# Kevindqz/hybrid-vehicle-platoon

Hardware: NVIDIA B200
Metric: hybrid-MPC solves/sec at n=10,N=6 (per-vehicle local MIQPs, proven optimal) (higher is better)
Workload: dtype f64

## Files before the change

hybrid_vehicle_platoon_b200/csrc/flat_core.cuh:

```cuda
#pragma once
#include <math.h>
#include <stdint.h>

#include "miqp_core.cuh"

#if defined(__CUDACC__)
#define HVP_ROLL _Pragma("unroll 1")
#define HVP_FLAT_UNROLL _Pragma("unroll")
#else
#define HVP_ROLL
#define HVP_FLAT_UNROLL
#endif
#if defined(__CUDA_ARCH__)
#define HVP_LDG(p) __ldg(p)
#else
#define HVP_LDG(p) (*(p))
#endif

namespace hvp {

#if defined(__CUDA_ARCH__)
extern __shared__ double hvp_flat_slab[];
#endif

HVP_HD double hvp_rcp(double v) {
#if defined(__CUDA_ARCH__)
    double r;
    asm("rcp.approx.ftz.f64 %0, %1;" : "=d"(r) : "d"(v));
    r = r * (2.0 - v * r);
    r = r * (2.0 - v * r);
    return r;
#else
    return 1.0 / v;
#endif
}

#ifdef HVP_DEBUG_STATS
static long g_it[16], g_nodes[16], g_q[16], g_st[4], g_warm[8];
#endif
template <int N>
struct FlatLayout {
    static constexpr int TRI = N * (N + 1) / 2;
    static constexpr int O_HINV = 0;
    static constexpr int O_GINV = N * N;
    static constexpr int O_X = O_GINV + TRI;
    static constexpr int O_LAM = O_X + N;
    static constexpr int O_YP = O_LAM + N;
    static constexpr int O_D = O_YP + N;
    static constexpr int O_WV = O_D;
    static constexpr int O_R = O_D + N;
    static constexpr int SIZE = O_R + N;
};

template <int N>
struct FlatCold {
    double gt[N], xstar[N], rlo[N + 1], rhi[N + 1], amax[N], amin[N];
    long long t_start;
    double pf[N + 1], pnz[N + 1], ptp[N + 1], ptm[N + 1];
};

template <int N, int ST, bool ALG2 = false, bool HINTS = false>
struct FlatSolver {
    using LY = FlatLayout<N>;
    enum : int { S_NEXT = 0, S_BUILD, S_SELECT, S_STEP, S_DONE };
    static constexpr bool kHull = false;

    double* W;
    const LocalParams* P;
    const double* xf_;
    const double* xb_;
    double* best_;
    FlatCold<N>* C;
    double p0, v0, pc, inv_m, a_lo, a_hi, c_lo, c_hi, hw1, hw2, hd, ct;
    bool has_sf, has_sb;
    double sfv[N], sbv[N];
    int state, lev, L, nodes, iters, it;
    double inc;
    uint64_t modes_pk, best_modes, cand_pk, built_pk;
    int built_L;
    bool trouble, limit, timeout;
    bool dive;
    bool hinted;
    int hint_c0;
    bool fresh;
#ifdef HVP_DEBUG_STATS
    bool was_warm = false;
#endif
    bool slab_ok;
    int q;
    uint64_t act_lo, act_hi;
    uint32_t satf, satb;
    int pid, pkind, pj;
    double psgn, pcoef, nHn, lam_p, cp;
    double dual;
    bool p_soft;

    int lane_;
    HVP_HD double& w(int off, int i) const {
#if defined(__CUDA_ARCH__)
        return hvp_flat_slab[(off + i) * ST + lane_];
#else
        return W[(size_t)(off + i) * ST];
#endif
    }
    HVP_HD static int tri(int a, int b) { return a * (a + 1) / 2 + b; }
    HVP_HD double ra(int rg) const { return rg < 4 ? a_lo : a_hi; }
    HVP_HD double rc(int rg) const { return rg < 4 ? c_lo : c_hi; }
    HVP_HD double rb(int rg) const { return P->bgear[rg] * inv_m; }
    HVP_HD static int mode_of(uint64_t pk, int k) { return (int)((pk >> (3 * k)) & 7u); }
    HVP_HD int mode(int k) const { return mode_of(modes_pk, k); }
    HVP_HD void set_mode(int k, int rg) { modes_pk = (modes_pk & ~(7ull << (3 * k))) | ((uint64_t)rg << (3 * k)); }
    HVP_HD int cand(int lv) const { return (int)((cand_pk >> (7 * lv)) & 0x7fu); }
    HVP_HD void set_cand(int lv, int v) { cand_pk = (cand_pk & ~(0x7full << (7 * lv))) | ((uint64_t)v << (7 * lv)); }
    HVP_HD int act_raw(int a) const { return (int)(((a < 8 ? act_lo >> (8 * a) : act_hi >> (8 * (a - 8)))) & 0xffu); }
    HVP_HD int act(int a) const { return act_raw(a) & 0x7f; }
    HVP_HD double slot_sgn(int a) const { return (act_raw(a) & 0x80) ? -1.0 : 1.0; }
    HVP_HD double slot_coef(int a) const {
        const int id = act(a), t = id / 12;
        return (t == T_UHI || t == T_ULO) ? ra(mode(id - 12 * t)) : 1.0;
    }
    HVP_HD void set_act(int a, int id) {
        if (a < 8) act_lo = (act_lo & ~(0xffull << (8 * a))) | ((uint64_t)id << (8 * a));
        else act_hi = (act_hi & ~(0xffull << (8 * (a - 8)))) | ((uint64_t)id << (8 * (a - 8)));
    }
    HVP_HD double Hoff(int j) const { return hw1 * (double)(N - 1 - j) + hw2; }
    HVP_HD double Hdiag(int j) const { return hw1 * (double)(N - 1 - j) + hd; }
    HVP_HD double sf(int j) const { return HVP_LDG(xf_ + j + 1) - P->d_safe - pc; }
    HVP_HD double sb(int j) const { return HVP_LDG(xb_ + j + 1) + P->d_safe - pc; }

    HVP_HD void setup(double* W_, const LocalParams* P_, int flags, double mass, const double* x0,
                      const double* xf, const double* xb, const double* xl, double* best_out, FlatCold<N>* cold) {
        W = W_; P = P_; xf_ = xf; xb_ = xb; best_ = best_out; C = cold;
        p0 = x0[0]; v0 = x0[1]; pc = p0 + v0;
        inv_m = hvp_rcp(mass);
        a_lo = 1.0 - P->c1 * inv_m; a_hi = 1.0 - P->c2 * inv_m;
        c_lo = -P->mug; c_hi = -P->mug - P->dfr * inv_m;
        const bool is_front = flags & 1, is_leader = flags & 2, is_trailer = flags & 4;
        const bool tf = !is_front && !is_leader, tb = !is_trailer && !is_leader, tl = is_leader;
        const double wp = P->qxp, wvv = P->qxv, t0 = P->t0, d0 = P->d0;
        const int np1 = N + 1;
        const double nterm = (tf ? 1.0 : 0.0) + (tb ? 1.0 : 0.0) + (tl ? 1.0 : 0.0);
        hw1 = 2.0 * wp * nterm;
        hw2 = 2.0 * wp * (tf ? t0 : 0.0);
        hd = 2.0 * wp * (tf ? t0 * t0 : 0.0) + 2.0 * wvv * nterm;
        HVP_ROLL
        for (int j = 0; j < N; ++j) C->gt[j] = 0.0;
        ct = 0.0;
        HVP_ROLL
        for (int kind = 0; kind < 3; ++kind) {
            const double* ref = kind == 0 ? xf : (kind == 1 ? xb : xl);
            const bool on = kind == 0 ? tf : (kind == 1 ? tb : tl);
            if (!on) continue;
            const double tau = kind == 0 ? t0 : 0.0;
            double suffix = 0.0;
            HVP_ROLL
            for (int k = N; k >= 0; --k) {
                const double pk = ref[k], vk = ref[np1 + k];
                const double Pk = (kind == 0) ? (pk - d0) : (kind == 1) ? (pk + t0 * vk + d0) : pk;
                if (k >= 1) {
                    const double rho = pc - Pk;
                    C->gt[k - 1] += 2.0 * wp * (suffix + tau * rho) - 2.0 * wvv * vk;
                    ct += wp * rho * rho + wvv * vk * vk;
                    suffix += rho;
                } else {
                    const double e0 = p0 + tau * v0 - Pk, e1 = v0 - vk;
                    ct += wp * e0 * e0 + wvv * e1 * e1;
                }
            }
        }
        has_sf = !is_front; has_sb = !is_trailer;
        const double ww = P->w, ds = P->d_safe;
        if (has_sf) {
            const double s0 = p0 - (xf[0] - ds), s1 = pc - (xf[1] - ds);
            ct += ww * (s0 > 0 ? s0 : 0.0) + ww * (s1 > 0 ? s1 : 0.0);
        }
        if (has_sb) {
            const double s0 = (xb[0] + ds) - p0, s1 = (xb[1] + ds) - pc;
            ct += ww * (s0 > 0 ? s0 : 0.0) + ww * (s1 > 0 ? s1 : 0.0);
        }
        HVP_FLAT_UNROLL
        for (int j = 1; j < N; ++j) {
            sfv[j] = has_sf ? sf(j) : 0.0;
            sbv[j] = has_sb ? sb(j) : 0.0;
        }
        sfv[0] = sbv[0] = 0.0;
        if (nterm > 0.5) {
            const double* h0 = P->h0inv[tf ? (tb ? 2 : 1) : 0];
            HVP_ROLL
            for (int e = 0; e < N * N; ++e) w(LY::O_HINV, e) = h0[e];
        } else {
            HVP_ROLL
            for (int i = 0; i < N; ++i) {
                HVP_ROLL
                for (int j = 0; j < N; ++j) w(LY::O_HINV, i * N + j) = (i == j) ? Hdiag(i) : Hoff(i > j ? i : j);
            }
            HVP_ROLL
            for (int k = 0; k < N; ++k) {
                const double pinv = hvp_rcp(w(LY::O_HINV, k * N + k));
                HVP_ROLL
                for (int j = 0; j < N; ++j) w(LY::O_HINV, k * N + j) *= pinv;
                w(LY::O_HINV, k * N + k) = pinv;
                HVP_ROLL
                for (int i = 0; i < N; ++i) {
                    if (i == k) continue;
                    const double f = w(LY::O_HINV, i * N + k);
                    HVP_ROLL
                    for (int j = 0; j < N; ++j)
                        w(LY::O_HINV, i * N + j) = (j == k) ? -f * pinv : w(LY::O_HINV, i * N + j) - f * w(LY::O_HINV, k * N + j);
                }
            }
        }
        built_L = 0; built_pk = 0;
        iters = 0; nodes = 0; it = 0; modes_pk = 0; best_modes = 0; cand_pk = 0;
        inc = HUGE_VAL; trouble = limit = timeout = false; lev = 0; dive = P->dive != 0; fresh = false; slab_ok = false;
        hinted = false;
        if (P->time_limit_ns > 0) C->t_start = hvp_now_ns();
        if (ALG2) C->pf[0] = -HUGE_VAL;
        int c0 = 0;
        HVP_ROLL
        for (int rg = 0; rg < NREG; ++rg)
            if (v0 >= P->edge[rg] && v0 <= P->edge[rg + 1]) c0 |= (1 << rg);
        set_cand(0, c0);
        C->xstar[0] = v0; C->rlo[0] = v0; C->rhi[0] = v0;
        state = S_NEXT;
    }

    HVP_HD void apply_hint(const int32_t* h) {
        const double eps = 1e-9;
        const int c0 = cand(0);
        bool ok = true;
        HVP_ROLL
        for (int lv = 0; lv < N && ok; ++lv) {
            const int rg = h[lv];
            int cn = c0;
            if (lv > 0) {
                cn = 0;
                HVP_ROLL
                for (int c = 0; c < NREG; ++c)
                    if (P->edge[c] <= C->rhi[lv] && P->edge[c + 1] >= C->rlo[lv]) cn |= (1 << c);
            }
            if (rg < 0 || rg >= NREG || !((cn >> rg) & 1)) { ok = false; break; }
            set_mode(lv, rg);
            set_cand(lv, cn & ~(1 << rg));
            const double jlo = fmax(C->rlo[lv], P->edge[rg]), jhi = fmin(C->rhi[lv], P->edge[rg + 1]);
            double nlo = fmax(ra(rg) * jlo + rc(rg) + rb(rg) * P->umin, jlo + P->a_dec + lv * P->tight);
            double nhi = fmin(ra(rg) * jhi + rc(rg) + rb(rg) * P->umax, jhi + P->a_acc - lv * P->tight);
            nlo = fmax(nlo, P->vmin); nhi = fmin(nhi, P->vmax);
            if (jlo > jhi + eps || nlo > nhi + eps) { ok = false; break; }
            if (lv + 1 < N) { C->rlo[lv + 1] = nlo - eps; C->rhi[lv + 1] = nhi + eps; C->xstar[lv + 1] = v0; }
        }
        if (!ok || pc > P->pmax + eps || pc < P->pmin - eps) { unhint(c0); return; }
        hint_c0 = c0;
        lev = N - 1;
        L = N;
        hinted = true;
        state = S_BUILD;
    }
    HVP_HD void unhint(int c0) {
        modes_pk = 0; cand_pk = 0;
        set_cand(0, c0);
        lev = 0;
        state = S_NEXT;
    }

    HVP_HD bool open_level(int& l, int& cb, int& total) const {
        l = -1; cb = 0; total = 0;
        HVP_ROLL
        for (int lv = 0; lv <= lev; ++lv) {
            const int c = cand(lv);
            if (c && l < 0) { l = lv; cb = c; }
            total += __builtin_popcount((unsigned)c);
        }
        return l >= 0;
    }
    HVP_HD void adopt_prefix(uint64_t donor_modes, int l, int c, double donor_inc) {
        const double eps = 1e-9;
        HVP_ROLL
        for (int lv = 0; lv < l; ++lv) {
            const int rg = mode_of(donor_modes, lv);
            set_mode(lv, rg);
            set_cand(lv, 0);
            const double jlo = fmax(C->rlo[lv], P->edge[rg]), jhi = fmin(C->rhi[lv], P->edge[rg + 1]);
            double nlo = fmax(ra(rg) * jlo + rc(rg) + rb(rg) * P->umin, jlo + P->a_dec + lv * P->tight);
            double nhi = fmin(ra(rg) * jhi + rc(rg) + rb(rg) * P->umax, jhi + P->a_acc - lv * P->tight);
            nlo = fmax(nlo, P->vmin); nhi = fmin(nhi, P->vmax);
            C->rlo[lv + 1] = nlo - eps; C->rhi[lv + 1] = nhi + eps;
            C->xstar[lv + 1] = v0;
            if (ALG2) C->pf[lv + 1] = -HUGE_VAL;
        }
        fresh = false; slab_ok = false;
        set_cand(l, 1 << c);
        lev = l;
        inc = donor_inc;
        dive = false;
        state = S_NEXT;
    }

    HVP_HD void parent_info() {
        const double ww = P->w, INF = HUGE_VAL;
        const int pj0 = lev - 1;
        HVP_ROLL
        for (int i = 0; i < N; ++i) w(LY::O_YP, i) = w(LY::O_HINV, pj0 * N + i);
        const double nHn0 = w(LY::O_HINV, pj0 * N + pj0);
        HVP_ROLL
        for (int a = 0; a < q; ++a) w(LY::O_D, a) = slot_dot(a, LY::O_YP);
        double nz = nHn0, tp = INF, tm = INF;
        HVP_ROLL
        for (int a = 0; a < q; ++a) {
            double s = 0.0;
            int gi = tri(a, 0);
            HVP_ROLL
            for (int b = 0; b <= a; ++b) s += w(LY::O_GINV, gi + b) * w(LY::O_D, b);
            gi += 2 * a + 1;
            HVP_ROLL
            for (int b = a + 1; b < q; ++b) { s += w(LY::O_GINV, gi) * w(LY::O_D, b); gi += b + 1; }
            nz -= s * w(LY::O_D, a);
            const double la = w(LY::O_LAM, a);
            const bool soft = act(a) >= T_SF * 12;
            if (s > 1e-14) {
                const double is = hvp_rcp(s);
                tp = fmin(tp, la * is);
                if (soft) tm = fmin(tm, (ww - la) * is);
            } else if (s < -1e-14) {
                const double is = hvp_rcp(-s);
                tm = fmin(tm, la * is);
                if (soft) tp = fmin(tp, (ww - la) * is);
            }
        }
        if (q == N || !(nz > 1e-11 * nHn0)) nz = 0.0;
        C->pnz[lev] = nz; C->ptp[lev] = fmax(tp, 0.0); C->ptm[lev] = fmax(tm, 0.0);
    }

    HVP_HD void do_next() {
        const double eps = 1e-9;
        if (ALG2 && fresh) { parent_info(); fresh = false; }
        for (;;) {
            int cset = cand(lev);
            if (cset == 0) {
                if (lev == 0) { state = S_DONE; return; }
                --lev;
                continue;
            }
            int rg = -1; double bd = HUGE_VAL;
            const double xs = C->xstar[lev];
            HVP_ROLL
            for (int c = 0; c < NREG; ++c) {
                if (!((cset >> c) & 1)) continue;
                const double lo = P->edge[c], hi = P->edge[c + 1];
                const double dist = xs < lo ? lo - xs : (xs > hi ? xs - hi : 0.0);
                if (dist < bd) { bd = dist; rg = c; }
            }
            set_cand(lev, cset & ~(1 << rg));
            const double pf = ALG2 ? C->pf[lev] : -HUGE_VAL;
            if (ALG2 && bd > 0.0 && inc < HUGE_VAL && pf > -HUGE_VAL && P->sibling_bound) {
                const double nz = C->pnz[lev];
                const double tmax = (xs > P->edge[rg + 1]) ? C->ptp[lev] : C->ptm[lev];
                const double t = (nz > 0.0) ? fmin(bd * hvp_rcp(nz), tmax) : tmax;
                const double bound = (t < HUGE_VAL) ? pf + t * bd - 0.5 * t * t * nz : HUGE_VAL;
                if (bound > inc) continue;
            }
            set_mode(lev, rg);
            const double jlo = fmax(C->rlo[lev], P->edge[rg]), jhi = fmin(C->rhi[lev], P->edge[rg + 1]);
            if (jlo > jhi + eps) continue;
            double nlo = fmax(ra(rg) * jlo + rc(rg) + rb(rg) * P->umin, jlo + P->a_dec + lev * P->tight);
            double nhi = fmin(ra(rg) * jhi + rc(rg) + rb(rg) * P->umax, jhi + P->a_acc - lev * P->tight);
            nlo = fmax(nlo, P->vmin); nhi = fmin(nhi, P->vmax);
            if (nlo > nhi + eps) continue;
            if (pc > P->pmax + eps || pc < P->pmin - eps) continue;
            C->rlo[lev + 1] = nlo - eps; C->rhi[lev + 1] = nhi + eps;
            L = lev + 1;
            if (dive && nodes >= 1 && L < N) {
                ++lev;
                C->xstar[lev] = w(LY::O_X, lev - 1);
                if (ALG2) C->pf[lev] = -HUGE_VAL;
                int cn = 0;
                HVP_ROLL
                for (int c = 0; c < NREG; ++c)
                    if (P->edge[c] <= C->rhi[lev] && P->edge[c + 1] >= C->rlo[lev]) cn |= (1 << c);
                set_cand(lev, cn);
                continue;
            }
            if (kHull) hull();
            state = S_BUILD;
            return;
        }
    }

    HVP_HD void hull() {
        const double eps = 1e-9;
        double lo = C->rlo[L], hi = C->rhi[L];
        HVP_ROLL
        for (int s = L; s < N; ++s) {
            double nlo = HUGE_VAL, nhi = -HUGE_VAL, dmax = -HUGE_VAL, dmin = HUGE_VAL;
            HVP_ROLL
            for (int r = 0; r < NREG; ++r) {
                const double jlo = fmax(lo, P->edge[r]), jhi = fmin(hi, P->edge[r + 1]);
                if (jlo > jhi + eps) continue;
                const double a = ra(r), b = rb(r), c = rc(r);
                nlo = fmin(nlo, a * jlo + c + b * P->umin);
                nhi = fmax(nhi, a * jhi + c + b * P->umax);
                dmax = fmax(dmax, (a - 1.0) * jlo + c + b * P->umax);
                dmin = fmin(dmin, (a - 1.0) * jhi + c + b * P->umin);
            }
            const double acc = P->a_acc - s * P->tight, dec = P->a_dec + s * P->tight;
            C->amax[s] = fmin(dmax + eps, acc); C->amin[s] = fmax(dmin - eps, dec);
            nlo = fmax(fmax(nlo, lo + dec), P->vmin); nhi = fmin(fmin(nhi, hi + acc), P->vmax);
            lo = nlo - eps; hi = nhi + eps;
            C->rlo[s + 1] = lo; C->rhi[s + 1] = hi;
        }
    }

    HVP_HD void node_done(int st, double obj) {
        iters += it;
        ++nodes;
#ifdef HVP_DEBUG_STATS
        g_it[L] += it; g_nodes[L] += 1; g_q[L] += q; g_st[st] += 1;
        if (was_warm) { g_warm[3] += it; } else { g_warm[4] += it; g_warm[5] += 1; } was_warm = false;
#endif
        state = S_NEXT;
        if (HINTS && hinted) {
            hinted = false;
            if (st != 0) { --nodes; unhint(hint_c0); return; }
            HVP_ROLL
            for (int lv = 1; lv < N; ++lv) C->xstar[lv] = w(LY::O_X, lv - 1);
        }
        if (st != 0 || L == N) dive = false;
        if (st == 2) { trouble = true; return; }
        if (st == 1) return;
        if (inc < HUGE_VAL && !(obj < hvp_cut(inc, P->mip_gap))) return;
        if (L == N) {
            inc = obj; best_modes = modes_pk;
            HVP_ROLL
            for (int j = 0; j < N; ++j) best_[j] = w(LY::O_X, j);
            return;
        }
        if (P->max_nodes > 0 && nodes >= P->max_nodes) { limit = true; state = S_DONE; return; }
        if (P->time_limit_ns > 0 && hvp_now_ns() - C->t_start > P->time_limit_ns) { timeout = true; state = S_DONE; return; }
        ++lev;
        C->xstar[lev] = w(LY::O_X, lev - 1);
        if (ALG2) { C->pf[lev] = fmin(obj, dual); fresh = true; slab_ok = true; }
        int cn = 0;
        HVP_ROLL
        for (int c = 0; c < NREG; ++c)
            if (P->edge[c] <= C->rhi[lev] && P->edge[c + 1] >= C->rlo[lev]) cn |= (1 << c);
        set_cand(lev, cn);
    }

    HVP_HD double rank1(int k, int rg, double s) {
        const double ib = hvp_rcp(rb(rg)), ea = (k >= 1) ? -ra(rg) * ib : 0.0;
        double ev = 0.0;
        HVP_ROLL
        for (int i = 0; i < N; ++i) {
            double v = ib * w(LY::O_HINV, i * N + k);
            if (k >= 1) v += ea * w(LY::O_HINV, i * N + k - 1);
            w(LY::O_WV, i) = v;
        }
        ev = ib * w(LY::O_WV, k) + ((k >= 1) ? ea * w(LY::O_WV, k - 1) : 0.0);
        const double den = hvp_rcp(1.0 / (2.0 * P->qu) * s + ev);
        double vr[N];
        HVP_FLAT_UNROLL
        for (int j = 0; j < N; ++j) vr[j] = w(LY::O_WV, j);
        HVP_ROLL
        for (int i = 0; i < N; ++i) {
            const double vi = w(LY::O_WV, i) * den;
            HVP_FLAT_UNROLL
            for (int j = 0; j < N; ++j) w(LY::O_HINV, i * N + j) -= vi * vr[j];
        }
        return den;
    }

    HVP_HD void do_build() {
        const double qu = P->qu, ww = P->w;
        int c = 0;
        while (c < built_L && c < L && mode_of(built_pk, c) == mode(c)) ++c;
        const bool warm = ALG2 && slab_ok && P->warm && L == built_L + 1 && c == built_L && (satf | satb) == 0u && q > 0;
        slab_ok = false;
        if (warm) {
            const double den = rank1(L - 1, mode(L - 1), 1.0);
            HVP_ROLL
            for (int a = 0; a < q; ++a) w(LY::O_R, a) = slot_dot(a, LY::O_WV);
            double zr = 0.0;
            HVP_ROLL
            for (int a = 0; a < q; ++a) {
                double s = 0.0;
                int gi = tri(a, 0);
                HVP_ROLL
                for (int b = 0; b <= a; ++b) s += w(LY::O_GINV, gi + b) * w(LY::O_R, b);
                gi += 2 * a + 1;
                HVP_ROLL
                for (int b = a + 1; b < q; ++b) { s += w(LY::O_GINV, gi) * w(LY::O_R, b); gi += b + 1; }
                w(LY::O_YP, a) = s;
                zr += s * w(LY::O_R, a);
            }
            const double alpha = den * hvp_rcp(1.0 - den * zr);
            HVP_ROLL
            for (int a = 0; a < q; ++a) {
                const double ra_ = alpha * w(LY::O_YP, a);
                HVP_ROLL
                for (int b = 0; b <= a; ++b) w(LY::O_GINV, tri(a, b)) += ra_ * w(LY::O_YP, b);
            }
        } else {
            HVP_ROLL
            for (int k = built_L - 1; k >= c; --k) rank1(k, mode_of(built_pk, k), -1.0);
            HVP_ROLL
            for (int k = c; k < L; ++k) rank1(k, mode(k), 1.0);
        }
        built_L = L; built_pk = modes_pk;
        HVP_ROLL
        for (int i = 0; i < N; ++i) w(LY::O_D, i) = C->gt[i];
        dual = ct;
        HVP_ROLL
        for (int k = 0; k < L; ++k) {
            const int rg = mode(k);
            const double ib = hvp_rcp(rb(rg)), ea = -ra(rg) * ib;
            const double kc = (k == 0) ? -(ra(rg) * v0 + rc(rg)) * ib : -rc(rg) * ib;
            w(LY::O_D, k) += 2.0 * qu * kc * ib;
            if (k >= 1) w(LY::O_D, k - 1) += 2.0 * qu * kc * ea;
            dual += qu * kc * kc;
        }
        double gr[N];
        HVP_FLAT_UNROLL
        for (int j = 0; j < N; ++j) gr[j] = w(LY::O_D, j);
        HVP_ROLL
        for (int i = 0; i < N; ++i) {
            double s = 0.0;
            HVP_FLAT_UNROLL
            for (int j = 0; j < N; ++j) s -= w(LY::O_HINV, i * N + j) * gr[j];
            if (ALG2) w(LY::O_R, i) = s - w(LY::O_X, i);
            w(LY::O_X, i) = s;
            dual += 0.5 * w(LY::O_D, i) * s;
        }
        it = 0; satf = 0; satb = 0;
        state = S_SELECT;
#ifdef HVP_DEBUG_STATS
        g_warm[0] += 1; if (warm) g_warm[1] += 1;
#endif
        if (warm) {
            HVP_ROLL
            for (int a = 0; a < q; ++a) {
                const int id = act(a), t = id / 12, j = id - 12 * t;
                double cv;
                if (t <= T_LB) {
                    double lo, hi;
                    bounds(j, lo, hi);
                    cv = (t == T_UB) ? w(LY::O_X, j) - hi : lo - w(LY::O_X, j);
                } else {
                    cv = slot_dot(a, LY::O_R);
                }
                w(LY::O_YP, a) = cv;
            }
            bool ok = true;
            double cl = 0.0;
            HVP_ROLL
            for (int a = 0; a < q; ++a) {
                double s = 0.0;
                int gi = tri(a, 0);
                HVP_ROLL
                for (int b = 0; b <= a; ++b) s += w(LY::O_GINV, gi + b) * w(LY::O_YP, b);
// ... 248 lines not shown
            const double is = hvp_rcp(nz);
            HVP_ROLL
            for (int a = 0; a < q; ++a) {
                const double ra_ = w(LY::O_R, a) * is;
                HVP_ROLL
                for (int b = 0; b <= a; ++b) w(LY::O_GINV, tri(a, b)) += ra_ * w(LY::O_R, b);
                w(LY::O_GINV, tri(q, a)) = -ra_;
            }
            w(LY::O_GINV, tri(q, q)) = is;
            set_act(q, pid | (psgn < 0.0 ? 0x80 : 0));
            w(LY::O_LAM, q) = lam_p;
            ++q;
            state = S_SELECT;
            return;
        }
        if (t == t3p) {
            if (pid / 12 == T_SF) satf ^= (1u << pj); else satb ^= (1u << pj);
            state = S_SELECT;
            return;
        }
        int drop;
        if (t == t1) drop = k1;
        else {
            drop = k3;
            const int id = act(drop), j = id % 12;
            if (id / 12 == T_SF) satf ^= (1u << j); else satb ^= (1u << j);
        }
        {
            const double ikk = hvp_rcp(w(LY::O_GINV, tri(drop, drop)));
            HVP_ROLL
            for (int a = 0; a < q; ++a) w(LY::O_D, a) = w(LY::O_GINV, a >= drop ? tri(a, drop) : tri(drop, a));
            HVP_ROLL
            for (int a = 0; a < q; ++a) {
                if (a == drop) continue;
                const int an = a > drop ? a - 1 : a;
                const double da = w(LY::O_D, a) * ikk;
                HVP_ROLL
                for (int b = 0; b <= a; ++b) {
                    if (b == drop) continue;
                    const int bn = b > drop ? b - 1 : b;
                    w(LY::O_GINV, tri(an, bn)) = w(LY::O_GINV, tri(a, b)) - da * w(LY::O_D, b);
                }
            }
        }
        HVP_ROLL
        for (int a = drop; a + 1 < q; ++a) {
            set_act(a, act_raw(a + 1));
            w(LY::O_LAM, a) = w(LY::O_LAM, a + 1);
        }
        --q;
    }

    HVP_HD void trip() {
        if (state == S_NEXT) do_next();
        if (state == S_BUILD) do_build();
        if (state == S_SELECT) do_select();
        if (state == S_STEP) do_step();
    }
    HVP_HD bool wants_node() const { return state == S_NEXT || state == S_BUILD; }
    HVP_HD void trip_node() {
        if (state == S_NEXT) do_next();
        if (state == S_BUILD) do_build();
    }
    HVP_HD void trip_step() {
        if (state == S_SELECT) do_select();
        if (state == S_STEP) do_step();
    }

    HVP_HD LocalResult finish(double* u_out, double* x_out, int32_t* mode_out) const {
        LocalResult R;
        R.nodes = nodes; R.qp_iters = iters;
        const int np1 = N + 1;
        if (inc < HUGE_VAL) {
            R.obj = inc;
            R.status = timeout ? HVP_ST_TIME_LIMIT : limit ? HVP_ST_NODE_LIMIT : (trouble ? HVP_ST_NUMERIC : HVP_ST_OPTIMAL);
            double p = p0, v = v0;
            x_out[0] = p; x_out[np1] = v;
            HVP_ROLL
            for (int k = 0; k < N; ++k) {
                const int rg = mode_of(best_modes, k);
                const double vn = x_out[np1 + k + 1];
                u_out[k] = (vn - ra(rg) * v - rc(rg)) / rb(rg);
                mode_out[k] = rg;
                p = p + v; v = vn;
                x_out[k + 1] = p;
            }
        } else {
            R.obj = HUGE_VAL;
            R.status = timeout ? HVP_ST_TIME_LIMIT : limit ? HVP_ST_NODE_LIMIT : (trouble ? HVP_ST_NUMERIC : HVP_ST_INFEASIBLE);
            HVP_ROLL
            for (int k = 0; k < N; ++k) { u_out[k] = 0.0; mode_out[k] = -1; }
            HVP_ROLL
            for (int k = 0; k <= N; ++k) { x_out[k] = 0.0; x_out[np1 + k] = 0.0; }
        }
        return R;
    }
};

}
```

hybrid_vehicle_platoon_b200/csrc/local_miqp.cu:

```cuda
#include <cuda_runtime.h>
#include <stdint.h>
#include <stdlib.h>
#include <string.h>

#include "coop_core.cuh"
#include "flat_core.cuh"
#include "hvp_internal.h"
#include "miqp_core.cuh"

namespace hvp {

template <int G>
__global__ void __launch_bounds__(COOP_BLOCK)
coop_miqp_kernel(const __grid_constant__ LocalParams P, int64_t batch, const int32_t* __restrict__ flags,
                 const double* __restrict__ mass, const double* __restrict__ x0,
                 const double* __restrict__ xf, const double* __restrict__ xb,
                 const double* __restrict__ xl, double* __restrict__ u, double* __restrict__ x,
                 int32_t* __restrict__ modes, double* __restrict__ obj, int32_t* __restrict__ status,
                 int32_t* __restrict__ nodes, int32_t* __restrict__ qp_iters, int spread) {
    const int64_t t = (int64_t)blockIdx.x * blockDim.x + threadIdx.x;
    if (spread && (threadIdx.x & 31) >= G) return;
    const int64_t i = spread ? (t >> 5) : t / G;
    if (i >= batch) return;
    const int N = P.N;
    const size_t S = 2 * (size_t)(N + 1);
    CoopSolver<DevBK<G>> sol;
    sol.setup(&P, flags[i], mass[i], x0 + 2 * i, xf ? xf + S * i : nullptr, xb ? xb + S * i : nullptr,
              xl ? xl + S * i : nullptr);
    const LocalResult R = sol.solve(u + (size_t)N * i, x + S * i, modes + (size_t)N * i);
    if (sol.bk.ln == 0) {
        obj[i] = R.obj;
        status[i] = R.status;
        nodes[i] = R.nodes;
        if (qp_iters) qp_iters[i] = R.qp_iters;
    }
}

constexpr int COOP_SPLIT_MAX = 64;
constexpr int COOP_SPLIT_ROW = 48;

template <int G>
__global__ void __launch_bounds__(32)
coop_split_kernel(const __grid_constant__ LocalParams P, int64_t batch, int M, const int32_t* __restrict__ flags,
                  const double* __restrict__ mass, const double* __restrict__ x0,
                  const double* __restrict__ xf, const double* __restrict__ xb,
                  const double* __restrict__ xl, double* __restrict__ u, double* __restrict__ x,
                  int32_t* __restrict__ modes, double* __restrict__ obj, int32_t* __restrict__ status,
                  int32_t* __restrict__ nodes, int32_t* __restrict__ qp_iters, unsigned* __restrict__ done,
                  unsigned long long* __restrict__ keys, double* __restrict__ rows) {
    if (threadIdx.x >= G) return;
    const int64_t i = blockIdx.x / M;
    const int w = blockIdx.x % M;
    const int N = P.N, np1 = N + 1;
    const size_t S = 2 * (size_t)np1;
    CoopSolver<DevBK<G>> sol;
    sol.setup(&P, flags[i], mass[i], x0 + 2 * i, xf ? xf + S * i : nullptr, xb ? xb + S * i : nullptr,
              xl ? xl + S * i : nullptr);
    sol.sub_M = M; sol.sub_w = w; sol.shared = keys + i;
    double* row = rows + ((size_t)i * M + w) * COOP_SPLIT_ROW;
    int32_t* rmodes = reinterpret_cast<int32_t*>(row + N + S);
    const LocalResult R = sol.solve(row, row + N, rmodes);
    const int ln = sol.bk.ln;
    unsigned old = 0;
    if (ln == 0) {
        double* tail = row + 2 * N + S;
        tail[0] = R.obj; tail[1] = (double)R.status; tail[2] = (double)R.nodes; tail[3] = (double)R.qp_iters;
    }
    __syncwarp((1u << G) - 1u);
    __threadfence();
    if (ln == 0) old = atomicAdd(done + i, 1u);
    old = __shfl_sync((1u << G) - 1u, old, 0);
    if (old != (unsigned)(M - 2)) return;
    __threadfence();
    double bv = HUGE_VAL;
    int bw = 0, nsum = 0, isum = 0;
    bool numeric = false, limited = false, timed = false;
    for (int c = 0; c < M; ++c) {
        const double* t = rows + ((size_t)i * M + c) * COOP_SPLIT_ROW + 2 * N + S;
        const double o = *reinterpret_cast<const volatile double*>(t);
        const int st = (int)*reinterpret_cast<const volatile double*>(t + 1);
        nsum += (int)*reinterpret_cast<const volatile double*>(t + 2);
        isum += (int)*reinterpret_cast<const volatile double*>(t + 3);
        if (o < bv) { bv = o; bw = c; }
        numeric = numeric || st == HVP_ST_NUMERIC; limited = limited || st == HVP_ST_NODE_LIMIT;
        timed = timed || st == HVP_ST_TIME_LIMIT;
    }
    const double* src = rows + ((size_t)i * M + bw) * COOP_SPLIT_ROW;
    const int32_t* smodes = reinterpret_cast<const int32_t*>(src + N + S);
    for (int e = ln; e < N; e += G) { u[(size_t)N * i + e] = src[e]; modes[(size_t)N * i + e] = smodes[e]; }
    for (int e = ln; e < (int)S; e += G) x[S * i + e] = src[N + e];
    if (ln == 0) {
        obj[i] = bv;
        status[i] = timed ? HVP_ST_TIME_LIMIT : limited ? HVP_ST_NODE_LIMIT
                          : (numeric ? HVP_ST_NUMERIC : (bv < HUGE_VAL ? HVP_ST_OPTIMAL : HVP_ST_INFEASIBLE));
        nodes[i] = nsum;
        if (qp_iters) qp_iters[i] = isum;
    }
}

template <int N, bool STEAL, bool HINTS>
__global__ void __launch_bounds__(32, (N <= 6 ? 10 : (N == 7 ? 7 : (N == 8 ? 6 : 5))))
flat_miqp_kernel(const __grid_constant__ LocalParams P, int64_t batch, const int32_t* __restrict__ flags,
                 const double* __restrict__ mass, const double* __restrict__ x0,
                 const double* __restrict__ xf, const double* __restrict__ xb,
                 const double* __restrict__ xl, double* __restrict__ u, double* __restrict__ x,
                 int32_t* __restrict__ modes, double* __restrict__ obj, int32_t* __restrict__ status,
                 int32_t* __restrict__ nodes, int32_t* __restrict__ qp_iters, unsigned long long* __restrict__ counter,
                 double* __restrict__ scratch) {
    extern __shared__ double smem[];
    using Solver = FlatSolver<N, 32, false, HINTS>;
    const int lane = threadIdx.x;
    const size_t S = 2 * (size_t)(N + 1);
    Solver sol;
    FlatCold<N> cold;
    sol.lane_ = lane;
    sol.P = &P;
    bool have = false;
    int64_t i = 0;
    const bool steal = STEAL && scratch != nullptr && P.max_nodes == 0;
    bool thief = false, drained = false;
    int owner = lane, pending = 0;
    double* const my_scratch = scratch ? scratch + ((size_t)blockIdx.x * 32 + lane) * N : nullptr;
    const int node_batch = P.node_batch;
    for (;;) {
        __syncwarp();
        const bool slow = !have || sol.state == Solver::S_DONE || sol.wants_node();
        const unsigned ms = __ballot_sync(0xffffffffu, slow);
        if (ms == 0xffffffffu || __popc(ms) >= node_batch) {
            if (STEAL && __builtin_expect(drained, 0)) {
                unsigned rep = __ballot_sync(0xffffffffu, have && thief && sol.state == Solver::S_DONE && pending == 0);
                while (rep) {
                    const int r = __ffs(rep) - 1;
                    rep &= rep - 1;
                    const int o = __shfl_sync(0xffffffffu, owner, r);
                    const double v = __shfl_sync(0xffffffffu, sol.inc, r);
                    const unsigned long long bm = __shfl_sync(0xffffffffu, (unsigned long long)sol.best_modes, r);
                    const int nn = __shfl_sync(0xffffffffu, sol.nodes, r), ii = __shfl_sync(0xffffffffu, sol.iters, r);
                    const int tr = __shfl_sync(0xffffffffu, (int)sol.trouble, r);
                    __syncwarp();
                    if (lane == o) {
                        --pending;
                        sol.nodes += nn; sol.iters += ii;
                        if (tr) sol.trouble = true;
                        if (v < sol.inc) {
                            sol.inc = v; sol.best_modes = bm;
                            const double* src = scratch + ((size_t)blockIdx.x * 32 + r) * N;
                            for (int j = 0; j < N; ++j) sol.best_[j] = src[j];
                        }
                    }
                    if (lane == r) { have = false; thief = false; owner = lane; }
                }
                __syncwarp();
            }
            if (have && !thief && sol.state == Solver::S_DONE && pending == 0) {
                const LocalResult R = sol.finish(u + (size_t)N * i, x + S * i, modes + (size_t)N * i);
                obj[i] = R.obj;
                status[i] = R.status;
                nodes[i] = R.nodes;
                if (qp_iters) qp_iters[i] = R.qp_iters;
                have = false;
            }
            bool start = false, adopting = false;
            int a_l = 0, a_c = 0, a_owner = lane;
            unsigned long long a_modes = 0;
            double a_inc = 0.0;
            const unsigned need = __ballot_sync(0xffffffffu, !have);
            if (need && !drained) {
                unsigned long long base = 0;
                if (lane == 0) base = atomicAdd(counter, (unsigned long long)__popc(need));
                base = __shfl_sync(0xffffffffu, base, 0);
                if (!have) {
                    const int64_t cand_i = (int64_t)base + __popc(need & ((1u << lane) - 1u));
                    if (cand_i < batch) { i = cand_i; start = true; }
                }
                if ((int64_t)base + __popc(need) > batch) drained = true;
            }
            if (STEAL && __builtin_expect(steal && drained, 0)) {
                const double oi = __shfl_sync(0xffffffffu, sol.inc, thief ? owner : lane);
                if (have && thief && oi < sol.inc) sol.inc = oi;
                unsigned idle = __ballot_sync(0xffffffffu, !have && !start);
                int l = -1, cb = 0, total = 0;
                const bool can = have && sol.state == Solver::S_NEXT && sol.open_level(l, cb, total) && total >= 2;
                unsigned don = __ballot_sync(0xffffffffu, can);
                for (int round = 0; round < 4 && don && idle; ++round) {
                    const int d = __ffs(don) - 1;
                    don &= don - 1;
                    const int dl = __shfl_sync(0xffffffffu, l, d), dcb = __shfl_sync(0xffffffffu, cb, d);
                    const int dtot = __shfl_sync(0xffffffffu, total, d);
                    const long long di = __shfl_sync(0xffffffffu, (long long)i, d);
                    const unsigned long long dm = __shfl_sync(0xffffffffu, (unsigned long long)sol.modes_pk, d);
                    const double dinc = __shfl_sync(0xffffffffu, sol.inc, d);
                    int m = __popc((unsigned)dcb) - (dtot == __popc((unsigned)dcb) ? 1 : 0);
                    if (m > __popc(idle)) m = __popc(idle);
                    if (m <= 0) continue;
                    const bool me_idle = (idle >> lane) & 1u;
                    const int rk = __popc(idle & ((1u << lane) - 1u));
                    if (me_idle && rk < m) {
                        int bits = dcb;
                        for (int t = 0; t < rk; ++t) bits &= bits - 1;
                        a_c = __ffs(bits) - 1; a_l = dl; a_modes = dm; a_inc = dinc; a_owner = d;
                        i = di; start = true; adopting = true;
                    }
                    if (lane == d) {
                        int bits = dcb, rm = 0;
                        for (int t = 0; t < m; ++t) { rm |= bits & -bits; bits &= bits - 1; }
                        sol.set_cand(dl, dcb & ~rm);
                        pending += m;
                    }
                    idle = __ballot_sync(0xffffffffu, !have && !start);
                }
            }
            if (start) {
                sol.setup(smem + lane, &P, flags[i], mass[i], x0 + 2 * i, xf ? xf + S * i : nullptr,
                          xb ? xb + S * i : nullptr, xl ? xl + S * i : nullptr,
                          adopting ? my_scratch : x + S * i + (N + 2), &cold);
                if (STEAL && adopting) sol.adopt_prefix(a_modes, a_l, a_c, a_inc);
                else if (HINTS && P.hint) sol.apply_hint(P.hint + (size_t)N * i);
                have = true; thief = adopting; owner = a_owner;
            }
            if (!__any_sync(0xffffffffu, have)) break;
            if (have) sol.trip_node();
        }
        if (have) sol.trip_step();
    }
}

static int env_int(const char* name, int dflt) {
    const char* e = getenv(name);
    return e ? atoi(e) : dflt;
}

template <int N>
static cudaError_t launch_flat(const LocalParams& P, unsigned long long* counter, double* steal_scratch, int64_t batch, const int32_t* flags, const double* mass,
                               const double* x0, const double* xf, const double* xb, const double* xl, double* u,
                               double* x, int32_t* modes, double* obj, int32_t* status, int32_t* nodes,
                               int32_t* qp_iters, cudaStream_t stream) {
    const size_t smem = (size_t)FlatLayout<N>::SIZE * 32 * sizeof(double);
    int dev = 0;
    cudaGetDevice(&dev);
    static int grid_cache[HVP_MAX_DEVICES] = {0};
    int uncached = 0;
    int& grid_full = (dev >= 0 && dev < HVP_MAX_DEVICES) ? grid_cache[dev] : uncached;
    if (!grid_full) {
        cudaError_t e = cudaSuccess;
        const void* fns[3] = {(const void*)flat_miqp_kernel<N, true, false>, (const void*)flat_miqp_kernel<N, false, false>,
                              (const void*)flat_miqp_kernel<N, true, true>};
        for (int v = 0; v < 3; ++v) {
            const void* fn = fns[v];
            e = cudaFuncSetAttribute(fn, cudaFuncAttributeMaxDynamicSharedMemorySize, (int)smem);
            if (e != cudaSuccess) return e;
            e = cudaFuncSetAttribute(fn, cudaFuncAttributePreferredSharedMemoryCarveout, cudaSharedmemCarveoutMaxShared);
            if (e != cudaSuccess) return e;
        }
        int sms = 0, per_sm = 0;
        cudaDeviceGetAttribute(&sms, cudaDevAttrMultiProcessorCount, dev);
        e = cudaOccupancyMaxActiveBlocksPerMultiprocessor(&per_sm, flat_miqp_kernel<N, true, false>, 32, smem);
        if (e != cudaSuccess) return e;
        grid_full = sms * (per_sm > 0 ? per_sm : 1);
    }
    int64_t g = (batch + 31) / 32;
    static const int gdiv = env_int("HVP_FLAT_GRID_DIV", 1);
    if (g > grid_full / gdiv) g = grid_full / gdiv;
    LocalParams Q = P;
    static const int nb = env_int("HVP_NODE_BATCH", 0), dv = env_int("HVP_FLAT_DIVE", -1);
    if (nb > 0) Q.node_batch = nb;
    if (dv >= 0) Q.dive = dv;
    static const int steal_on = env_int("HVP_FLAT_STEAL", 1);
    if ((size_t)g * 32 * N > HVP_STEAL_SLOT_DOUBLES) steal_scratch = nullptr;
    cudaError_t e = cudaMemsetAsync(counter, 0, sizeof(unsigned long long), stream);
    if (e != cudaSuccess) return e;
    if (Q.hint)
        flat_miqp_kernel<N, true, true><<<(unsigned)g, 32, smem, stream>>>(Q, batch, flags, mass, x0, xf, xb, xl, u, x, modes, obj,
                                                                          status, nodes, qp_iters, counter,
                                                                          steal_on ? steal_scratch : nullptr);
    else if (steal_on && steal_scratch)
        flat_miqp_kernel<N, true, false><<<(unsigned)g, 32, smem, stream>>>(Q, batch, flags, mass, x0, xf, xb, xl, u, x, modes, obj,
                                                                           status, nodes, qp_iters, counter, steal_scratch);
    else
        flat_miqp_kernel<N, false, false><<<(unsigned)g, 32, smem, stream>>>(Q, batch, flags, mass, x0, xf, xb, xl, u, x, modes, obj,
                                                                            status, nodes, qp_iters, counter, nullptr);
    return cudaGetLastError();
}

static int kernel_choice() {
    static int v = -1;
    if (v < 0) {
        const char* e = getenv("HVP_LOCAL_KERNEL");
        v = 0;
        if (e && strcmp(e, "coop") == 0) v = 2;
        if (e && strcmp(e, "flat") == 0) v = 3;
    }
    return v;
}

cudaError_t launch_local_miqp(const LocalParams& P, unsigned long long* counter, double* steal_scratch, int64_t batch, const int32_t* flags, const double* mass,
                              const double* x0, const double* xf, const double* xb, const double* xl,
                              double* u, double* x, int32_t* modes, double* obj, int32_t* status,
                              int32_t* nodes, int32_t* qp_iters, cudaStream_t stream) {
    if (batch <= 0) return cudaSuccess;
    const int choice = kernel_choice();
    const bool flat_ok = P.N >= 4 && P.N <= 9;
    if (flat_ok && (choice == 3 || (choice == 0 && batch >= FLAT_MIN_BATCH))) {
#define HVP_FLAT(NN) case NN: return launch_flat<NN>(P, counter, steal_scratch, batch, flags, mass, x0, xf, xb, xl, u, x, modes, obj, status, nodes, qp_iters, stream);
        switch (P.N) { HVP_FLAT(4) HVP_FLAT(5) HVP_FLAT(6) HVP_FLAT(7) HVP_FLAT(8) HVP_FLAT(9) default: break; }
#undef HVP_FLAT
    }
    {
        static const int splitM = env_int("HVP_COOP_SPLIT_M", 8);
        if (P.N <= 8 && batch <= COOP_SPLIT_MAX && splitM > 1 && splitM <= 32 && steal_scratch && P.max_nodes == 0 &&
            2 * P.N + 2 * (P.N + 1) + 4 <= COOP_SPLIT_ROW) {
            const size_t head = (size_t)COOP_SPLIT_MAX * (sizeof(unsigned) + sizeof(unsigned long long));
            unsigned* done = reinterpret_cast<unsigned*>(steal_scratch);
            unsigned long long* keys = reinterpret_cast<unsigned long long*>(reinterpret_cast<char*>(steal_scratch) + COOP_SPLIT_MAX * sizeof(unsigned));
            double* rows = reinterpret_cast<double*>(reinterpret_cast<char*>(steal_scratch) + head);
            cudaError_t e = cudaMemsetAsync(steal_scratch, 0xFF, head, stream);
            if (e != cudaSuccess) return e;
            coop_split_kernel<8><<<(unsigned)(batch * splitM), 32, 0, stream>>>(P, batch, splitM, flags, mass, x0, xf, xb, xl, u, x,
                                                                                modes, obj, status, nodes, qp_iters, done, keys, rows);
            return cudaGetLastError();
        }
        if (P.N <= 8) {
            if (batch <= COOP_SPREAD_MAX) {
                coop_miqp_kernel<8><<<(unsigned)batch, 32, 0, stream>>>(P, batch, flags, mass, x0, xf, xb, xl, u, x, modes,
// ... 25 lines not shown
```

Baseline: 37.95 million.

## Defer node-open/leaf work into settle state to reduce warp divergence

Introduces deferred S_OPEN and S_LEAF states so that opening a child level (candidate-set computation, xstar update) and copying an incumbent leaf happen in a common settle() step, not inside node_done. This is meant to lower lane divergence in the warp-lockstep branch-and-bound loop. Candidate sets are now pre-filtered by interval feasibility, and do_next jumps to the deepest open level with a bitmask MSB instead of walking up level by level. The incremental rebuild finds the shared mode prefix via XOR/LSB and merges the remove/add rank-1 loops into one. Debug counters are added behind a compile flag, and the new state machine risks subtle ordering bugs with stealing and hints.

```diff
diff --git a/hybrid_vehicle_platoon_b200/csrc/flat_core.cuh b/hybrid_vehicle_platoon_b200/csrc/flat_core.cuh
--- a/hybrid_vehicle_platoon_b200/csrc/flat_core.cuh
+++ b/hybrid_vehicle_platoon_b200/csrc/flat_core.cuh
@@ -35,8 +35,33 @@
 #endif
 }
 
+HVP_HD int hvp_msb64(uint64_t v) {
+#if defined(__CUDA_ARCH__)
+    return 63 - __clzll((long long)v);
+#else
+    return 63 - __builtin_clzll(v);
+#endif
+}
+HVP_HD int hvp_lsb64(uint64_t v) {
+#if defined(__CUDA_ARCH__)
+    return __ffsll((long long)v) - 1;
+#else
+    return __builtin_ctzll(v);
+#endif
+}
+
 #ifdef HVP_DEBUG_STATS
 static long g_it[16], g_nodes[16], g_q[16], g_st[4], g_warm[8];
+#endif
+enum { CTR_SETUP = 0, CTR_NEXT, CTR_BUILD, CTR_NODE_DONE, CTR_SETTLE, CTR_FINISH, CTR_FUNCS };
+#if defined(HVP_FLAT_COUNTERS) && defined(__CUDA_ARCH__)
+#define HVP_CTR(k)                                                                    \
+    {                                                                                 \
+        const unsigned am__ = __activemask();                                         \
+        if (__ffs(am__) - 1 == lane_) { C->ctr[2 * (k)] += 1; C->ctr[2 * (k) + 1] += __popc(am__); } \
+    }
+#else
+#define HVP_CTR(k)
 #endif
 template <int N>
 struct FlatLayout {
@@ -57,12 +82,15 @@
     double gt[N], xstar[N], rlo[N + 1], rhi[N + 1], amax[N], amin[N];
     long long t_start;
     double pf[N + 1], pnz[N + 1], ptp[N + 1], ptm[N + 1];
+#ifdef HVP_FLAT_COUNTERS
+    unsigned long long ctr[2 * CTR_FUNCS];
+#endif
 };
 
 template <int N, int ST, bool ALG2 = false, bool HINTS = false>
 struct FlatSolver {
     using LY = FlatLayout<N>;
-    enum : int { S_NEXT = 0, S_BUILD, S_SELECT, S_STEP, S_DONE };
+    enum : int { S_NEXT = 0, S_BUILD, S_SELECT, S_STEP, S_DONE, S_OPEN, S_LEAF };
     static constexpr bool kHull = false;
 
     double* W;
@@ -131,6 +159,7 @@
     HVP_HD void setup(double* W_, const LocalParams* P_, int flags, double mass, const double* x0,
                       const double* xf, const double* xb, const double* xl, double* best_out, FlatCold<N>* cold) {
         W = W_; P = P_; xf_ = xf; xb_ = xb; best_ = best_out; C = cold;
+        HVP_CTR(CTR_SETUP);
         p0 = x0[0]; v0 = x0[1]; pc = p0 + v0;
         inv_m = hvp_rcp(mass);
         a_lo = 1.0 - P->c1 * inv_m; a_hi = 1.0 - P->c2 * inv_m;
@@ -216,40 +245,47 @@
         hinted = false;
         if (P->time_limit_ns > 0) C->t_start = hvp_now_ns();
         if (ALG2) C->pf[0] = -HUGE_VAL;
-        int c0 = 0;
-        HVP_ROLL
-        for (int rg = 0; rg < NREG; ++rg)
-            if (v0 >= P->edge[rg] && v0 <= P->edge[rg + 1]) c0 |= (1 << rg);
-        set_cand(0, c0);
         C->xstar[0] = v0; C->rlo[0] = v0; C->rhi[0] = v0;
-        state = S_NEXT;
+        state = S_OPEN;
+    }
+
+    HVP_HD bool interval(int lv, int rg, double& nlo, double& nhi) const {
+        const double eps = 1e-9;
+        const double jlo = fmax(C->rlo[lv], P->edge[rg]), jhi = fmin(C->rhi[lv], P->edge[rg + 1]);
+        nlo = fmax(ra(rg) * jlo + rc(rg) + rb(rg) * P->umin, jlo + P->a_dec + lv * P->tight);
+        nhi = fmin(ra(rg) * jhi + rc(rg) + rb(rg) * P->umax, jhi + P->a_acc - lv * P->tight);
+        nlo = fmax(nlo, P->vmin); nhi = fmin(nhi, P->vmax);
+        return !(jlo > jhi + eps) && !(nlo > nhi + eps);
+    }
+    HVP_HD int feasible_set(int lv) const {
+        const double eps = 1e-9;
+        if (pc > P->pmax + eps || pc < P->pmin - eps) return 0;
+        int cn = 0;
+        HVP_ROLL
+        for (int c = 0; c < NREG; ++c) {
+            double nlo, nhi;
+            if (P->edge[c] <= C->rhi[lv] && P->edge[c + 1] >= C->rlo[lv] && interval(lv, c, nlo, nhi)) cn |= (1 << c);
+        }
+        return cn;
     }
 
     HVP_HD void apply_hint(const int32_t* h) {
         const double eps = 1e-9;
+        settle();
         const int c0 = cand(0);
         bool ok = true;
         HVP_ROLL
         for (int lv = 0; lv < N && ok; ++lv) {
             const int rg = h[lv];
-            int cn = c0;
-            if (lv > 0) {
-                cn = 0;
-                HVP_ROLL
-                for (int c = 0; c < NREG; ++c)
-                    if (P->edge[c] <= C->rhi[lv] && P->edge[c + 1] >= C->rlo[lv]) cn |= (1 << c);
-            }
+            const int cn = lv > 0 ? feasible_set(lv) : c0;
             if (rg < 0 || rg >= NREG || !((cn >> rg) & 1)) { ok = false; break; }
             set_mode(lv, rg);
             set_cand(lv, cn & ~(1 << rg));
-            const double jlo = fmax(C->rlo[lv], P->edge[rg]), jhi = fmin(C->rhi[lv], P->edge[rg + 1]);
-            double nlo = fmax(ra(rg) * jlo + rc(rg) + rb(rg) * P->umin, jlo + P->a_dec + lv * P->tight);
-            double nhi = fmin(ra(rg) * jhi + rc(rg) + rb(rg) * P->umax, jhi + P->a_acc - lv * P->tight);
-            nlo = fmax(nlo, P->vmin); nhi = fmin(nhi, P->vmax);
-            if (jlo > jhi + eps || nlo > nhi + eps) { ok = false; break; }
+            double nlo, nhi;
+            interval(lv, rg, nlo, nhi);
             if (lv + 1 < N) { C->rlo[lv + 1] = nlo - eps; C->rhi[lv + 1] = nhi + eps; C->xstar[lv + 1] = v0; }
         }
-        if (!ok || pc > P->pmax + eps || pc < P->pmin - eps) { unhint(c0); return; }
+        if (!ok) { unhint(c0); return; }
         hint_c0 = c0;
         lev = N - 1;
         L = N;
@@ -266,7 +302,7 @@
     HVP_HD bool open_level(int& l, int& cb, int& total) const {
         l = -1; cb = 0; total = 0;
         HVP_ROLL
-        for (int lv = 0; lv <= lev; ++lv) {
+        for (int lv = 0; lv <= lev - (state == S_OPEN ? 1 : 0); ++lv) {
             const int c = cand(lv);
             if (c && l < 0) { l = lv; cb = c; }
             total += __builtin_popcount((unsigned)c);
@@ -280,10 +316,8 @@
             const int rg = mode_of(donor_modes, lv);
             set_mode(lv, rg);
             set_cand(lv, 0);
-            const double jlo = fmax(C->rlo[lv], P->edge[rg]), jhi = fmin(C->rhi[lv], P->edge[rg + 1]);
-            double nlo = fmax(ra(rg) * jlo + rc(rg) + rb(rg) * P->umin, jlo + P->a_dec + lv * P->tight);
-            double nhi = fmin(ra(rg) * jhi + rc(rg) + rb(rg) * P->umax, jhi + P->a_acc - lv * P->tight);
-            nlo = fmax(nlo, P->vmin); nhi = fmin(nhi, P->vmax);
+            double nlo, nhi;
+            interval(lv, rg, nlo, nhi);
             C->rlo[lv + 1] = nlo - eps; C->rhi[lv + 1] = nhi + eps;
             C->xstar[lv + 1] = v0;
             if (ALG2) C->pf[lv + 1] = -HUGE_VAL;
@@ -333,14 +367,14 @@
 
     HVP_HD void do_next() {
         const double eps = 1e-9;
+        HVP_CTR(CTR_NEXT);
         if (ALG2 && fresh) { parent_info(); fresh = false; }
         for (;;) {
-            int cset = cand(lev);
-            if (cset == 0) {
-                if (lev == 0) { state = S_DONE; return; }
-                --lev;
-                continue;
-            }
+            settle();
+            const uint64_t open = cand_pk & (~0ull >> (64 - 7 * (lev + 1)));
+            if (open == 0) { lev = 0; state = S_DONE; return; }
+            lev = hvp_msb64(open) / 7;
+            const int cset = cand(lev);
             int rg = -1; double bd = HUGE_VAL;
             const double xs = C->xstar[lev];
             HVP_ROLL
@@ -360,24 +394,14 @@
                 if (bound > inc) continue;
             }
             set_mode(lev, rg);
-            const double jlo = fmax(C->rlo[lev], P->edge[rg]), jhi = fmin(C->rhi[lev], P->edge[rg + 1]);
-            if (jlo > jhi + eps) continue;
-            double nlo = fmax(ra(rg) * jlo + rc(rg) + rb(rg) * P->umin, jlo + P->a_dec + lev * P->tight);
-            double nhi = fmin(ra(rg) * jhi + rc(rg) + rb(rg) * P->umax, jhi + P->a_acc - lev * P->tight);
-            nlo = fmax(nlo, P->vmin); nhi = fmin(nhi, P->vmax);
-            if (nlo > nhi + eps) continue;
-            if (pc > P->pmax + eps || pc < P->pmin - eps) continue;
+            double nlo, nhi;
+            interval(lev, rg, nlo, nhi);
             C->rlo[lev + 1] = nlo - eps; C->rhi[lev + 1] = nhi + eps;
             L = lev + 1;
             if (dive && nodes >= 1 && L < N) {
                 ++lev;
-                C->xstar[lev] = w(LY::O_X, lev - 1);
                 if (ALG2) C->pf[lev] = -HUGE_VAL;
-                int cn = 0;
-                HVP_ROLL
-                for (int c = 0; c < NREG; ++c)
-                    if (P->edge[c] <= C->rhi[lev] && P->edge[c + 1] >= C->rlo[lev]) cn |= (1 << c);
-                set_cand(lev, cn);
+                state = S_OPEN;
                 continue;
             }
             if (kHull) hull();
@@ -411,6 +435,7 @@
     }
 
     HVP_HD void node_done(int st, double obj) {
+        HVP_CTR(CTR_NODE_DONE);
         iters += it;
         ++nodes;
 #ifdef HVP_DEBUG_STATS
@@ -430,20 +455,26 @@
         if (inc < HUGE_VAL && !(obj < hvp_cut(inc, P->mip_gap))) return;
         if (L == N) {
             inc = obj; best_modes = modes_pk;
-            HVP_ROLL
-            for (int j = 0; j < N; ++j) best_[j] = w(LY::O_X, j);
+            state = S_LEAF;
             return;
         }
         if (P->max_nodes > 0 && nodes >= P->max_nodes) { limit = true; state = S_DONE; return; }
         if (P->time_limit_ns > 0 && hvp_now_ns() - C->t_start > P->time_limit_ns) { timeout = true; state = S_DONE; return; }
         ++lev;
-        C->xstar[lev] = w(LY::O_X, lev - 1);
         if (ALG2) { C->pf[lev] = fmin(obj, dual); fresh = true; slab_ok = true; }
-        int cn = 0;
-        HVP_ROLL
-        for (int c = 0; c < NREG; ++c)
-            if (P->edge[c] <= C->rhi[lev] && P->edge[c + 1] >= C->rlo[lev]) cn |= (1 << c);
-        set_cand(lev, cn);
+        state = S_OPEN;
+    }
+    HVP_HD void settle() {
+        if (state < S_OPEN) return;
+        HVP_CTR(CTR_SETTLE);
+        if (state == S_LEAF) {
+            HVP_ROLL
+            for (int j = 0; j < N; ++j) best_[j] = w(LY::O_X, j);
+        } else {
+            if (lev > 0) C->xstar[lev] = w(LY::O_X, lev - 1);
+            set_cand(lev, feasible_set(lev));
+        }
+        state = S_NEXT;
     }
 
     HVP_HD double rank1(int k, int rg, double s) {
@@ -471,8 +502,10 @@
 
     HVP_HD void do_build() {
         const double qu = P->qu, ww = P->w;
-        int c = 0;
-        while (c < built_L && c < L && mode_of(built_pk, c) == mode(c)) ++c;
+        HVP_CTR(CTR_BUILD);
+        const uint64_t diff = built_pk ^ modes_pk;
+        int c = built_L < L ? built_L : L;
+        if (diff) { const int k = hvp_lsb64(diff) / 3; if (k < c) c = k; }
         const bool warm = ALG2 && slab_ok && P->warm && L == built_L + 1 && c == built_L && (satf | satb) == 0u && q > 0;
         slab_ok = false;
         if (warm) {
@@ -500,10 +533,13 @@
                 for (int b = 0; b <= a; ++b) w(LY::O_GINV, tri(a, b)) += ra_ * w(LY::O_YP, b);
             }
         } else {
-            HVP_ROLL
-            for (int k = built_L - 1; k >= c; --k) rank1(k, mode_of(built_pk, k), -1.0);
-            HVP_ROLL
-            for (int k = c; k < L; ++k) rank1(k, mode(k), 1.0);
+            const int down = built_L - c, ops = down + L - c;
+            HVP_ROLL
+            for (int t = 0; t < ops; ++t) {
+                const bool rm = t < down;
+                const int k = rm ? built_L - 1 - t : c + t - down;
+                rank1(k, mode_of(rm ? built_pk : modes_pk, k), rm ? -1.0 : 1.0);
+            }
         }
         built_L = L; built_pk = modes_pk;
         HVP_ROLL
@@ -858,14 +894,15 @@
     }
 
     HVP_HD void trip() {
-        if (state == S_NEXT) do_next();
+        if (state == S_NEXT || state > S_DONE) do_next();
         if (state == S_BUILD) do_build();
         if (state == S_SELECT) do_select();
         if (state == S_STEP) do_step();
-    }
-    HVP_HD bool wants_node() const { return state == S_NEXT || state == S_BUILD; }
+        settle();
+    }
+    HVP_HD bool wants_node() const { return state == S_NEXT || state == S_BUILD || state > S_DONE; }
     HVP_HD void trip_node() {
-        if (state == S_NEXT) do_next();
+        if (state == S_NEXT || state > S_DONE) do_next();
         if (state == S_BUILD) do_build();
     }
     HVP_HD void trip_step() {
@@ -875,6 +912,7 @@
 
     HVP_HD LocalResult finish(double* u_out, double* x_out, int32_t* mode_out) const {
         LocalResult R;
+        HVP_CTR(CTR_FINISH);
         R.nodes = nodes; R.qp_iters = iters;
         const int np1 = N + 1;
         if (inc < HUGE_VAL) {
diff --git a/hybrid_vehicle_platoon_b200/csrc/local_miqp.cu b/hybrid_vehicle_platoon_b200/csrc/local_miqp.cu
--- a/hybrid_vehicle_platoon_b200/csrc/local_miqp.cu
+++ b/hybrid_vehicle_platoon_b200/csrc/local_miqp.cu
@@ -2,6 +2,9 @@
 #include <stdint.h>
 #include <stdlib.h>
 #include <string.h>
+#ifdef HVP_FLAT_COUNTERS
+#include <stdio.h>
+#endif
 
 #include "coop_core.cuh"
 #include "flat_core.cuh"
@@ -98,6 +101,10 @@
     }
 }
 
+#ifdef HVP_FLAT_COUNTERS
+__device__ unsigned long long hvp_flat_ctr[2 + 2 * CTR_FUNCS];
+#endif
+
 template <int N, bool STEAL, bool HINTS>
 __global__ void __launch_bounds__(32, (N <= 6 ? 10 : (N == 7 ? 7 : (N == 8 ? 6 : 5))))
 flat_miqp_kernel(const __grid_constant__ LocalParams P, int64_t batch, const int32_t* __restrict__ flags,
@@ -120,12 +127,18 @@
     const bool steal = STEAL && scratch != nullptr && P.max_nodes == 0;
     bool thief = false, drained = false;
     int owner = lane, pending = 0;
-    double* const my_scratch = scratch ? scratch + ((size_t)blockIdx.x * 32 + lane) * N : nullptr;
     const int node_batch = P.node_batch;
+#ifdef HVP_FLAT_COUNTERS
+    long long cyc_node = 0, cyc_step = 0, t_mark = clock64();
+    for (int k = 0; k < 2 * CTR_FUNCS; ++k) cold.ctr[k] = 0;
+#endif
     for (;;) {
         __syncwarp();
         const bool slow = !have || sol.state == Solver::S_DONE || sol.wants_node();
         const unsigned ms = __ballot_sync(0xffffffffu, slow);
+#ifdef HVP_FLAT_COUNTERS
+        { const long long t = clock64(); cyc_step += t - t_mark; t_mark = t; }
+#endif
         if (ms == 0xffffffffu || __popc(ms) >= node_batch) {
             if (STEAL && __builtin_expect(drained, 0)) {
                 unsigned rep = __ballot_sync(0xffffffffu, have && thief && sol.state == Solver::S_DONE && pending == 0);
@@ -144,6 +157,7 @@
                         if (tr) sol.trouble = true;
                         if (v < sol.inc) {
                             sol.inc = v; sol.best_modes = bm;
+                            if (sol.state == Solver::S_LEAF) sol.state = Solver::S_NEXT;
                             const double* src = scratch + ((size_t)blockIdx.x * 32 + r) * N;
                             for (int j = 0; j < N; ++j) sol.best_[j] = src[j];
                         }
@@ -180,7 +194,8 @@
                 if (have && thief && oi < sol.inc) sol.inc = oi;
                 unsigned idle = __ballot_sync(0xffffffffu, !have && !start);
                 int l = -1, cb = 0, total = 0;
-                const bool can = have && sol.state == Solver::S_NEXT && sol.open_level(l, cb, total) && total >= 2;
+                const bool can = have && (sol.state == Solver::S_NEXT || sol.state > Solver::S_DONE) &&
+                                 sol.open_level(l, cb, total) && total >= 2;
                 unsigned don = __ballot_sync(0xffffffffu, can);
                 for (int round = 0; round < 4 && don && idle; ++round) {
                     const int d = __ffs(don) - 1;
@@ -213,16 +228,31 @@
             if (start) {
                 sol.setup(smem + lane, &P, flags[i], mass[i], x0 + 2 * i, xf ? xf + S * i : nullptr,
                           xb ? xb + S * i : nullptr, xl ? xl + S * i : nullptr,
-                          adopting ? my_scratch : x + S * i + (N + 2), &cold);
+                          adopting ? scratch + ((size_t)blockIdx.x * 32 + lane) * N : x + S * i + (N + 2), &cold);
                 if (STEAL && adopting) sol.adopt_prefix(a_modes, a_l, a_c, a_inc);
                 else if (HINTS && P.hint) sol.apply_hint(P.hint + (size_t)N * i);
                 have = true; thief = adopting; owner = a_owner;
             }
             if (!__any_sync(0xffffffffu, have)) break;
             if (have) sol.trip_node();
+#ifdef HVP_FLAT_COUNTERS
+            __syncwarp();
+            { const long long t = clock64(); cyc_node += t - t_mark; t_mark = t; }
+#endif
         }
         if (have) sol.trip_step();
     }
+#ifdef HVP_FLAT_COUNTERS
+    for (int k = 0; k < 2 * CTR_FUNCS; ++k) {
+        unsigned long long v = cold.ctr[k];
+        for (int o = 16; o > 0; o >>= 1) v += __shfl_xor_sync(0xffffffffu, v, o);
+        if (lane == 0) atomicAdd(&hvp_flat_ctr[2 + k], v);
+    }
+    if (lane == 0) {
+        atomicAdd(&hvp_flat_ctr[0], (unsigned long long)cyc_node);
+        atomicAdd(&hvp_flat_ctr[1], (unsigned long long)cyc_step);
+    }
+#endif
 }
 
 static int env_int(const char* name, int dflt) {
@@ -269,6 +299,25 @@
     if ((size_t)g * 32 * N > HVP_STEAL_SLOT_DOUBLES) steal_scratch = nullptr;
     cudaError_t e = cudaMemsetAsync(counter, 0, sizeof(unsigned long long), stream);
     if (e != cudaSuccess) return e;
+#ifdef HVP_FLAT_COUNTERS
+    void* ctr = nullptr;
+    e = cudaGetSymbolAddress(&ctr, hvp_flat_ctr);
+    if (e != cudaSuccess) return e;
+    e = cudaMemsetAsync(ctr, 0, sizeof(hvp_flat_ctr), stream);
+    if (e != cudaSuccess) return e;
+    struct Report {
+        void* ctr; cudaStream_t s; int64_t batch;
+        ~Report() {
+            unsigned long long h[2 + 2 * CTR_FUNCS];
+            if (cudaMemcpyAsync(h, ctr, sizeof(h), cudaMemcpyDeviceToHost, s) != cudaSuccess || cudaStreamSynchronize(s) != cudaSuccess) return;
+            printf("HVP_FLAT_COUNTERS {\"batch\": %lld, \"cyc_node\": %llu, \"cyc_step\": %llu", (long long)batch, h[0], h[1]);
+            static const char* names[CTR_FUNCS] = {"setup", "next", "build", "node_done", "settle", "finish"};
+            for (int k = 0; k < CTR_FUNCS; ++k) printf(", \"%s\": [%llu, %llu]", names[k], h[2 + 2 * k], h[3 + 2 * k]);
+            printf("}\n");
+            fflush(stdout);
+        }
+    } report{ctr, stream, batch};
+#endif
     if (Q.hint)
         flat_miqp_kernel<N, true, true><<<(unsigned)g, 32, smem, stream>>>(Q, batch, flags, mass, x0, xf, xb, xl, u, x, modes, obj,
                                                                           status, nodes, qp_iters, counter,
```

Result: slower. 36.85 million, median of 6 (-2.9%).
